# Perception4D/LidarSlam

Measured on AMD Instinct MI355X. Metric: LiDAR frames/sec (AddFrame end-to-end), VLS-128 scan, higher is better.
Workload: dtype f32+f64; 1 GPU; VLS-128 synthetic spinning scan, street canyon, 5 m/s, EgoMotion=MOTION_EXTRAPOLATION_AND_REGISTRATION, Undistortion=REFINED, library defaults; points_per_frame=255802, sequences=1, parallelism=1 sequence per GPU x 1, frames_resident_in_hbm=False

## Files before the change

### lidarslam_amd/csrc/lsa_accum.h

```cpp
#pragma once
#include "lsa_ctx.h"

namespace lsa
{

struct RotConst
{
  double R[9], dRx[9], dRy[9], dRz[9];
  double t[3];
};
struct RecordSet
{
  const double* rec[3];
  const uint8_t* status[3];
  int count[3];
  int cap[3];
  double sat2[3];
};
struct AccumConst
{
  RotConst rot;
  RecordSet set;
  int jac;
};
// ... 60 lines not shown
  const double s = (r0 * r0 + r1 * r1) + r2 * r2;
  double rho0, rho1;
  if (s <= a2)
  {
    const double value = 1.0 - s / a2;
    const double value_sq = value * value;
    rho0 = a2 / 3.0 * (1.0 - value_sq * value);
    rho1 = value_sq;
  }
  else { rho0 = a2 / 3.0; rho1 = 0.0; }
  rho0 *= weight; rho1 *= weight;
  acc[0] += 0.5 * rho0;
  acc[28] += 1.0;
  if (!jac) return;
  double J[3][6];
#pragma unroll
  for (int a = 0; a < 3; ++a)
#pragma unroll
    for (int b = 0; b < 3; ++b) J[a][b] = A[a * 3 + b];
  double vx, vy, vz, cx, cy, cz;
  mv3(c.dRx, Xx, Xy, Xz, vx, vy, vz); mv3(A, vx, vy, vz, cx, cy, cz); J[0][3] = cx; J[1][3] = cy; J[2][3] = cz;
  mv3(c.dRy, Xx, Xy, Xz, vx, vy, vz); mv3(A, vx, vy, vz, cx, cy, cz); J[0][4] = cx; J[1][4] = cy; J[2][4] = cz;
  mv3(c.dRz, Xx, Xy, Xz, vx, vy, vz); mv3(A, vx, vy, vz, cx, cy, cz); J[0][5] = cx; J[1][5] = cy; J[2][5] = cz;
  int h = 7;
#pragma unroll
  for (int a = 0; a < 6; ++a)
  {
    acc[1 + a] += rho1 * ((J[0][a] * r0 + J[1][a] * r1) + J[2][a] * r2);
#pragma unroll
    for (int b = a; b < 6; ++b) acc[h++] += rho1 * ((J[0][a] * J[0][b] + J[1][a] * J[1][b]) + J[2][a] * J[2][b]);
  }
}

__device__ __forceinline__ void accumulate_records(const RecordSet& rs, const RotConst& c, bool jac, int first, int stride, double acc[kAccumVals])
{
  const int total = rs.count[0] + rs.count[1] + rs.count[2];
  for (int gidx = first; gidx < total; gidx += stride)
  {
    int t = 0, i = gidx;
    if (i >= rs.count[0]) { i -= rs.count[0]; t = 1; if (i >= rs.count[1]) { i -= rs.count[1]; t = 2; } }
    if (rs.status[t][i] != LSA_MATCH_SUCCESS) continue;
    const double* rec = rs.rec[t];
    const size_t cap = (size_t)rs.cap[t];
    double A[9];
#pragma unroll
    for (int f = 0; f < 9; ++f) A[f] = rec[f * cap + i];
    const double Px = rec[9 * cap + i], Py = rec[10 * cap + i], Pz = rec[11 * cap + i];
    const double Xx = rec[12 * cap + i], Xy = rec[13 * cap + i], Xz = rec[14 * cap + i];
    const double weight = rec[15 * cap + i];
    accumulate_one(A, Px, Py, Pz, Xx, Xy, Xz, weight, rs.sat2[t], c, jac, acc);
  }
}

struct RecordRegs
{
  double v[16];
  double a2;
  int state;
};
__device__ __forceinline__ void record_load(const RecordSet& rs, int gidx, RecordRegs& r)
{
  const int total = rs.count[0] + rs.count[1] + rs.count[2];
  r.state = -1;
  r.a2 = 0.;
#pragma unroll
  for (int f = 0; f < 16; ++f) r.v[f] = 0.;
  if (gidx >= total) return;
  int t = 0, i = gidx;
  if (i >= rs.count[0]) { i -= rs.count[0]; t = 1; if (i >= rs.count[1]) { i -= rs.count[1]; t = 2; } }
  const double* rec = rs.rec[t];
  const size_t cap = (size_t)rs.cap[t];
  const uint8_t st = rs.status[t][i];
#pragma unroll
  for (int f = 0; f < 16; ++f) r.v[f] = rec[f * cap + i];
  r.a2 = rs.sat2[t];
  r.state = st == LSA_MATCH_SUCCESS ? 1 : 0;
}
__device__ __forceinline__ void record_stash(const RecordRegs& r, double* __restrict__ cache, int cstride, int at)
{
  if (r.state == 1)
  {
#pragma unroll
    for (int f = 0; f < 16; ++f) cache[f * cstride + at] = r.v[f];
    cache[16 * cstride + at] = r.a2;
  }
  else if (r.state == 0)
    cache[15 * cstride + at] = -1.;
}

__device__ __forceinline__ void accumulate_records_cached(const RecordSet& rs, const RotConst& c, int first, int stride, double* __restrict__ cache,
                                                          int cslots, int cstride, bool fill, int prefilled, double acc[kAccumVals])
{
  const int total = rs.count[0] + rs.count[1] + rs.count[2];
  int j = 0;
  for (int gidx = first; gidx < total; gidx += stride, ++j)
  {
    double A[9], Px, Py, Pz, Xx, Xy, Xz, weight, a2;
    const int at = j * (int)blockDim.x + (int)threadIdx.x;
    if (j < cslots && (!fill || j < prefilled))
    {
      weight = cache[15 * cstride + at];
      if (weight < 0.) continue;
#pragma unroll
      for (int f = 0; f < 9; ++f) A[f] = cache[f * cstride + at];
      Px = cache[9 * cstride + at]; Py = cache[10 * cstride + at]; Pz = cache[11 * cstride + at];
      Xx = cache[12 * cstride + at]; Xy = cache[13 * cstride + at]; Xz = cache[14 * cstride + at];
      a2 = cache[16 * cstride + at];
    }
    else
    {
      int t = 0, i = gidx;
      if (i >= rs.count[0]) { i -= rs.count[0]; t = 1; if (i >= rs.count[1]) { i -= rs.count[1]; t = 2; } }
      if (rs.status[t][i] != LSA_MATCH_SUCCESS)
      {
        if (j < cslots) cache[15 * cstride + at] = -1.;
        continue;
      }
      const double* rec = rs.rec[t];
      const size_t cap = (size_t)rs.cap[t];
#pragma unroll
      for (int f = 0; f < 9; ++f) A[f] = rec[f * cap + i];
      Px = rec[9 * cap + i]; Py = rec[10 * cap + i]; Pz = rec[11 * cap + i];
      Xx = rec[12 * cap + i]; Xy = rec[13 * cap + i]; Xz = rec[14 * cap + i];
      weight = rec[15 * cap + i];
      a2 = rs.sat2[t];
      if (j < cslots)
      {
#pragma unroll
        for (int f = 0; f < 9; ++f) cache[f * cstride + at] = A[f];
// ... 64 lines not shown
```

### lidarslam_amd/csrc/lsa_lm.hip

```cpp
#include <chrono>
#include <cmath>
#include "lsa_accum.h"
#include "lsa_device_math.h"
#include "lsa_sensor_terms.h"
#include "../../include/lsa_pmath.h"

using namespace lsa;

namespace
{

typedef unsigned long long u64;
#ifndef LSA_RECORD_PREFETCH
#define LSA_RECORD_PREFETCH 1
#endif
constexpr bool kRecordPrefetch = LSA_RECORD_PREFETCH != 0;

struct LmParams
{
  RecordSet set;
  double x0[6];
  int two_d;
  int max_iter;
  int min_matches;
  unsigned tag_base;
  int cslots;
  int give_up_block;
  const IcpLinkBlock* link;
  IcpLinkBlock* leave;
  int link_refine;
  int motion_from_args;
  posemath::ScanPoseClock clock;
  Rigid previous_world;
  double motion0[16];
  double* motion_dev;
  lsa_sensor_terms_t sensors;
  int sensors_on;
};

constexpr int kResPose = 0, kResInitial = 6, kResFinal = 7, kResSums = 8, kResSuccessful = 37, kResUnsuccessful = 38, kResIterations = 39,
              kResEvaluations = 40, kResSkipped = 41, kResCode = 42, kResMatches = 43, kResFailed = 44, kResCount = 45;
static_assert(kResCount <= kLmOut, "result does not fit the mailbox");

__device__ __forceinline__ constexpr int hidx(int a, int b) { return 7 + a * 6 - (a * (a - 1)) / 2 + (b - a); }
__device__ __forceinline__ constexpr int hsym(int a, int b) { return a <= b ? hidx(a, b) : hidx(b, a); }

struct LmState
{
  int cur_buf;
  double x[6], scale[6], diag[6];
  double radius, decrease_factor, x_norm, model_cost_change, delta_norm, initial_cost;
  int reuse_diagonal, consecutive_invalid, iter;
  int evaluations, successful, unsuccessful, iterations, code, skipped, matches;
};

struct Shared
{
  double wsum[kLmThreads / 64][kAccumVals];
  double part[kAccumVals][8];
  double sums[2][kAccumVals];
  double Hs[36], gs[6];
  double w[6];
  double rot[39];
  LmState lm;
  int failed;
  int stop;
  unsigned long long lap[6], tk;
  unsigned long long sub[4], st0;
};

__device__ __forceinline__ double uniform(double v)
{
  const long long b = __double_as_longlong(v);
  const int lo = __builtin_amdgcn_readfirstlane((int)(b & 0xffffffffll)), hi = __builtin_amdgcn_readfirstlane((int)(b >> 32));
  return __longlong_as_double(((long long)hi << 32) | (long long)(unsigned)lo);
}

__device__ __forceinline__ double lane_value(double v, int lane)
{
  const long long b = __double_as_longlong(v);
  const int lo = __shfl((int)(b & 0xffffffffll), lane), hi = __shfl((int)(b >> 32), lane);
  return __longlong_as_double(((long long)hi << 32) | (long long)(unsigned)lo);
}

__device__ __forceinline__ double lane_bcast(double v, int src)
{
  const long long b = __double_as_longlong(v);
  const int lo = __builtin_amdgcn_readlane((int)(b & 0xffffffffll), src), hi = __builtin_amdgcn_readlane((int)(b >> 32), src);
  return __longlong_as_double(((long long)hi << 32) | (long long)(unsigned)lo);
}

__device__ __forceinline__ void lm_lap(Shared& sh, int slot)
{
  if (threadIdx.x == 0)
  {
    const unsigned long long now = wall_clock64();
    sh.lap[slot] += now - sh.tk;
    sh.tk = now;
  }
}

__device__ __noinline__ void lm_sensor_terms(const lsa_sensor_terms_t* terms, Shared& sh)
{
  sensor_terms_add(*terms, sh.w, sh.rot, sh.rot + 9, sh.rot + 18, sh.rot + 27, true, sh.sums[1 - sh.lm.cur_buf]);
}

__device__ __forceinline__ bool lm_evaluate(const LmParams& p, unsigned epoch, u64* __restrict__ xchg, Shared& sh, double* __restrict__ cache, bool trace)
{
  {
    RotConst c;
#pragma unroll
    for (int i = 0; i < 9; ++i) { c.R[i] = uniform(sh.rot[i]); c.dRx[i] = uniform(sh.rot[9 + i]); c.dRy[i] = uniform(sh.rot[18 + i]); c.dRz[i] = uniform(sh.rot[27 + i]); }
#pragma unroll
    for (int i = 0; i < 3; ++i) c.t[i] = uniform(sh.rot[36 + i]);
    double acc[kAccumVals];
#pragma unroll
    for (int v = 0; v < kAccumVals; ++v) acc[v] = 0.;
    const unsigned long long e0 = trace ? wall_clock64() : 0ull;
    accumulate_records_cached(p.set, c, blockIdx.x * blockDim.x + threadIdx.x, gridDim.x * blockDim.x, cache, p.cslots, p.cslots * kLmThreads, epoch == 1, kRecordPrefetch && p.cslots > 0 ? 1 : 0, acc);
    const unsigned long long e1 = trace ? wall_clock64() : 0ull;
    int slot;
    const double total = wave_reduce_accum(acc, slot);
    if (trace && threadIdx.x == 0) { sh.lap[4] += e1 - e0; }
    if ((threadIdx.x & 1) == 0 && slot < kAccumVals) sh.wsum[threadIdx.x >> 6][slot] = total;
  }
  if (threadIdx.x == 0) sh.failed = 0;
  __syncthreads();
  if (trace) lm_lap(sh, 0);
  const unsigned tag = p.tag_base + epoch;
  const int nb = gridDim.x;
  u64* slots = xchg + (size_t)(epoch & 1u) * kLmBlocksMax * kMailboxStride;
  if (threadIdx.x < 2 * kAccumVals)
  {
    const int v = threadIdx.x >> 1, half = threadIdx.x & 1;
    double r = sh.wsum[0][v];
#pragma unroll
    for (int w = 1; w < kLmThreads / 64; ++w) r += sh.wsum[w][v];
    const u64 bits = (u64)__double_as_longlong(r);
    const unsigned word = half ? (unsigned)(bits >> 32) : (unsigned)(bits & 0xffffffffull);
    __hip_atomic_store(slots + (size_t)blockIdx.x * kMailboxStride + threadIdx.x, ((u64)tag << 32) | word, __ATOMIC_RELAXED, __HIP_MEMORY_SCOPE_AGENT);
  }
  static_assert(kLmThreads / 64 == 8, "a wavefront per partial sum of the fold");
// ... 318 lines not shown
    {
      cand[lm_act<N>(a)] = x[lm_act<N>(a)] + step[a] * scale[a];
      const double e = x[lm_act<N>(a)] - cand[lm_act<N>(a)];
      dn += e * e;
    }
    delta_norm = __builtin_sqrt(dn);
    ++evaluations;
    break;
  }

  if (lane < N) lm.diag[lane] = diag_row;
  if (l0)
  {
    if (use_tot && !first)
    {
#pragma unroll
      for (int a = 0; a < 6; ++a) lm.x[a] = x[a];
    }
    lm.cur_buf = cur_buf;
    lm.x_norm = x_norm; lm.radius = radius; lm.decrease_factor = decrease_factor;
    lm.model_cost_change = model_cost_change; lm.delta_norm = delta_norm;
    lm.reuse_diagonal = reuse_diagonal; lm.consecutive_invalid = consecutive_invalid;
    lm.iter = iter; lm.iterations = iter;
    lm.successful = successful; lm.unsuccessful = unsuccessful; lm.evaluations = evaluations;
    lm.code = code;
    sh.stop = code != kCodeNone ? 1 : 0;
  }
  stamp(3);
  return code != kCodeNone;
}

__device__ void leave_link(const LmParams& p, const LmState& lm, bool failed, int part)
{
  using namespace posemath;
  IcpLinkBlock* g = p.leave;
  const int lane = threadIdx.x & 63;
  const bool go = !failed && !lm.skipped && lm.successful != 1;
  if (!go)
  {
    if (lane == 0 && part == 0) g->go = 0ull;
    return;
  }
  if (part == 1 && !p.link_refine) return;
  const double half = lm.x[3 + (lane < 6 ? lane % 3 : 0)] * 0.5;
  const double v = lane < 3 ? lsa_cos(half) : lsa_sin(half);
  const double cx = lane_value(v, 0), cy = lane_value(v, 1), cz = lane_value(v, 2);
  const double sx = lane_value(v, 3), sy = lane_value(v, 4), sz = lane_value(v, 5);
  double x[6];
#pragma unroll
  for (int a = 0; a < 6; ++a) x[a] = lm.x[a];
  const Pose T = FromXYZRPYTrig(x, cx, sx, cy, sy, cz, sz);
  if (part == 0)
  {
    if (lane != 0) return;
    double x0[6];
    ToXYZRPY(T, x0);
    g->in.pose = ToRigid(T);
#pragma unroll
    for (int a = 0; a < 6; ++a) g->in.x0[a] = x0[a];
    g->go = 1ull;
    return;
  }
  WithinFrameMotion m;
  double mv[16];
#pragma unroll
  for (int i = 0; i < 16; ++i) mv[i] = p.motion0[i];
  if (!p.motion_from_args)
  {
#pragma unroll
    for (int i = 0; i < 16; ++i) mv[i] = p.motion_dev[i];
  }
  m.Time0 = mv[0]; m.Time1 = mv[1];
  m.Rot0 = {mv[2], mv[3], mv[4], mv[5]};
  m.Rot1 = {mv[6], mv[7], mv[8], mv[9]};
#pragma unroll
  for (int i = 0; i < 3; ++i) { m.Trans0[i] = mv[10 + i]; m.Trans1[i] = mv[13 + i]; }
  const Pose previous = FromRigid(p.previous_world);
  const Pose mine = InterpolateScanPose(p.clock, previous, T, lane == 1 ? m.Time1 : m.Time0);
  Pose worldToBaseEnd = Pose::Identity();
#pragma unroll
  for (int i = 0; i < 3; ++i)
#pragma unroll
    for (int j = 0; j < 4; ++j) worldToBaseEnd(i, j) = lane_value(mine(i, j), 1);
  if (lane != 0) return;
  Pose d0, d1;
  RefineUndistortionFrom(m, mine, worldToBaseEnd, T, d0, d1);
  g->in.ic = MakeInterpConst(d0, d1, m.Time0, m.Time1);
  double* o = p.motion_dev;
  o[0] = m.Time0; o[1] = m.Time1;
  o[2] = m.Rot0.w; o[3] = m.Rot0.x; o[4] = m.Rot0.y; o[5] = m.Rot0.z;
  o[6] = m.Rot1.w; o[7] = m.Rot1.x; o[8] = m.Rot1.y; o[9] = m.Rot1.z;
#pragma unroll
  for (int i = 0; i < 3; ++i) { o[10 + i] = m.Trans0[i]; o[13 + i] = m.Trans1[i]; }
}

__global__ __launch_bounds__(kLmThreads) void k_lm_solve(LmParams p, u64* __restrict__ xchg, u64* __restrict__ mailbox, unsigned out_tag, unsigned long long* trace)
{
  __shared__ Shared sh;
  extern __shared__ double lm_cache[];
  const bool tr = trace != nullptr && blockIdx.x == 0;
  RecordRegs pre;
  if (kRecordPrefetch && p.cslots > 0) record_load(p.set, blockIdx.x * blockDim.x + threadIdx.x, pre);
  if (p.link)
  {
    if (p.link->go != 1ull)
    {
      if (p.leave && blockIdx.x == 0 && threadIdx.x == 0) p.leave->go = 0ull;
      return;
    }
  }
  if (threadIdx.x < 64)
  {
    double x0[6];
#pragma unroll
    for (int a = 0; a < 6; ++a) x0[a] = p.x0[a];
    if (p.link)
    {
#pragma unroll
      for (int a = 0; a < 6; ++a) x0[a] = p.link->in.x0[a];
    }
    if (threadIdx.x == 0)
    {
      for (int i = 0; i < 6; ++i) sh.lap[i] = 0;
      for (int i = 0; i < 4; ++i) sh.sub[i] = 0;
      sh.st0 = 0;
      sh.tk = wall_clock64();
      sh.lap[5] = sh.tk;
      LmState& lm = sh.lm;
#pragma unroll
      for (int v = 0; v < kAccumVals; ++v) sh.sums[0][v] = 0.;
      lm.cur_buf = 0;
#pragma unroll
      for (int a = 0; a < 6; ++a) { lm.x[a] = x0[a]; lm.scale[a] = 1.; lm.diag[a] = 0.; }
      lm.radius = 1e4; lm.decrease_factor = 2.0; lm.x_norm = 0.; lm.model_cost_change = 0.; lm.delta_norm = 0.; lm.initial_cost = 0.;
      lm.reuse_diagonal = 0; lm.consecutive_invalid = 0; lm.iter = 0;
      lm.evaluations = 1; lm.successful = 0; lm.unsuccessful = 0; lm.iterations = 0; lm.code = kCodeNone; lm.skipped = 0; lm.matches = 0;
      sh.stop = 0;
    }
    finish_point(sh, x0[0], x0[1], x0[2], x0[3], x0[4], x0[5]);
  }
  if (kRecordPrefetch && p.cslots > 0) record_stash(pre, lm_cache, p.cslots * kLmThreads, threadIdx.x);
  __syncthreads();
  bool failed = false;
  for (unsigned epoch = 1;; ++epoch)
  {
    if (!lm_evaluate(p, epoch, xchg, sh, lm_cache, tr)) { failed = true; break; }
    if (threadIdx.x < 64)
    {
      if (threadIdx.x == 0 && tr) sh.st0 = wall_clock64();
      double cand[6];
      const bool stop = p.two_d ? lm_step<3>(p, sh, epoch == 1, cand) : lm_step<6>(p, sh, epoch == 1, cand);
      if (!stop) finish_point(sh, cand[0], cand[1], cand[2], cand[3], cand[4], cand[5]);
    }
    __syncthreads();
    if (tr) lm_lap(sh, 3);
    if (sh.stop) break;
  }
  if (blockIdx.x != 0) return;
  if (tr && threadIdx.x == 0)
  {
    for (int i = 0; i < 4; ++i) trace[i] += sh.lap[i];
    trace[4] += (unsigned long long)sh.lm.evaluations;
    trace[5] += wall_clock64() - sh.lap[5];
    trace[6] += 1;
    trace[7] += sh.lap[4];
    for (int i = 0; i < 4; ++i) trace[8 + i] += sh.sub[i];
  }
  if (p.leave && threadIdx.x >= 64 && threadIdx.x < 192) leave_link(p, sh.lm, failed, (threadIdx.x >> 6) - 1);
  if (threadIdx.x < 2 * kResCount)
  {
    const LmState& lm = sh.lm;
    const int v = threadIdx.x >> 1, half = threadIdx.x & 1;
// ... 525 lines not shown
```

### lidarslam_amd/csrc/lsa_match_fused.hip

```cpp
#include <cmath>
#include "lsa_knn.h"
#include "lsa_match_internal.h"

using namespace lsa;

namespace
{

constexpr int kPending = -2;
constexpr int kShells = 7;
#ifndef LSA_KFILL
#define LSA_KFILL 3
#endif
#ifndef LSA_KHEAVY
#define LSA_KHEAVY 192
#endif
constexpr int kFill = LSA_KFILL;
constexpr int kHeavyCandidates = LSA_KHEAVY;

__device__ __forceinline__ constexpr int shell_level(int s) { return s < 2 ? 0 : (s < 4 ? 1 : 2); }
__device__ __forceinline__ constexpr int shell_r(int s) { return s == 6 ? 3 : ((s & 1) ? 2 : 1); }

template <int G>
__device__ __forceinline__ unsigned group_sum(unsigned v)
// ... 250 lines not shown
        const float dx = qx - cur[u].x, dy = qy - cur[u].y, dz = qz - cur[u].z;
        L.insert(make_key((dx * dx + dy * dy) + dz * dz, __float_as_int(cur[u].w)));
      }
  }
  if (route)
  {
    atomicAdd(&route[2], walked);
    atomicMax(&route[5], walked);
  }
}

template <int KMAX>
__device__ __forceinline__ void scan_heavy_blocks(unsigned long long pending, int G, const RowTable tb, knn_key* save, const float4* s0, const float4* s1,
                                               const float4* s2, int cur, int cbase, int nent, unsigned cand, float qx, float qy, float qz, int k, int* route)
{
  const int tid = threadIdx.x, lane = tid & 63;
  while (pending)
  {
    const int lead = __ffsll((long long)pending) - 1;
    pending &= pending - 1;
    const int hcur = __shfl(cur, lead), hbase = __shfl(cbase, lead), hnent = __shfl(nent, lead);
    const unsigned hcand = (unsigned)__shfl((int)cand, lead);
    const float hx = __shfl(qx, lead), hy = __shfl(qy, lead), hz = __shfl(qz, lead);
    const float4* hsorted = hcur < 2 ? s0 : (hcur < 4 ? s1 : s2);
    knn_key* const hslot = save + (size_t)(((tid & ~63) + lead) / G) * KMAX;
    LaneList<KMAX> H;
    H.reset();
    scan_rows<KMAX, 64>(H, tb, hbase, hnent, hcand, lane, hsorted, hx, hy, hz, nullptr);
#pragma unroll
    for (int s = 0; s < KMAX; ++s)
    {
      knn_key m = kKeyEmpty;
      if (s < k)
      {
        m = H.v[0];
        group_min<64>(m);
        if (H.v[0] == m)
        {
#pragma unroll
          for (int j = 0; j + 1 < KMAX; ++j) H.v[j] = H.v[j + 1];
          H.v[KMAX - 1] = kKeyEmpty;
        }
      }
      if (lane == 0) hslot[s] = m;
    }
    if (route && lane == 0) atomicAdd(&route[2], (int)hcand);
  }
  asm volatile("s_waitcnt lgkmcnt(0)" ::: "memory");
}

enum { kOutNone = 0, kOutFound = 1, kOutFar = 2, kOutTail = 3 };

template <int KMAX, int G>
__device__ __forceinline__ int group_search(const GridDesc* __restrict__ desc, const GridPtrs& gp, float qx, float qy, float qz, int k, float far_d2,
                                            bool active, int gl, int tid, const RowTable& tb, knn_key* save, knn_key (&best)[KMAX], float& ub_out, int* route,
                                            unsigned long long* phase = nullptr)
{
  auto stamp = [&](int i) { if (phase && (tid & 63) == 0) phase[(tid >> 6) * 8 + i] = wall_clock64(); };
  constexpr int E1 = (9 + G - 1) / G, E2 = (25 + G - 1) / G, E3 = (49 + G - 1) / G;
  constexpr int CAP = table_capacity<G>();
  static_assert((256 / G) * CAP <= kTableEntries, "row tables");
  const int gbase = ((tid - gl) / G) * CAP;
  const int base3[3] = {gbase, gbase + G * E1 + 1, gbase + G * (E1 + E2) + 2};
  const GridDesc g0 = desc[0], g1 = desc[1], g2 = desc[2];
  LevelView v0, v1, v2;
  level_view(v0, g0, qx, qy, qz);
  level_view(v1, g1, qx, qy, qz);
  level_view(v2, g2, qx, qy, qz);
  auto bound2 = [&](int s) {
    const int l = shell_level(s), r = shell_r(s);
    return l == 0 ? proven2(g0, v0, r) : (l == 1 ? proven2(g1, v1, r) : proven2(g2, v2, r));
  };
  auto fetch_any = [&](int s, bool live, bool& covered) -> unsigned {
    const int l = shell_level(s), r = shell_r(s);
    const GridDesc& g = l == 0 ? g0 : (l == 1 ? g1 : g2);
    const LevelView& v = l == 0 ? v0 : (l == 1 ? v1 : v2);
    const uint32_t* cs = l == 0 ? gp.cell_start[0] : (l == 1 ? gp.cell_start[1] : gp.cell_start[2]);
    uint32_t b[E3], en[E3];
    shell_rows<G, E3>(g, cs, v, r, gl, live, b, en, covered);
    return store_rows<G, E3>(tb, gbase, gl, live, b, en);
  };

  int outcome = kOutNone;
  int sh = -1, base = gbase;
  unsigned total = 0;
  bool sh_covered = false;
  bool need = active;
  ub_out = INFINITY;

  unsigned tot3[3];
  {
    uint32_t b0[E1], e0[E1], b1[E2], e1[E2], b2[E1], e2[E1];
    bool c0, c1, c2;
    shell_rows<G, E1>(g0, gp.cell_start[0], v0, 1, gl, active, b0, e0, c0);
    shell_rows<G, E2>(g0, gp.cell_start[0], v0, 2, gl, active, b1, e1, c1);
    shell_rows<G, E1>(g1, gp.cell_start[1], v1, 1, gl, active, b2, e2, c2);
    tot3[0] = store_rows<G, E1>(tb, base3[0], gl, active, b0, e0);
    tot3[1] = store_rows<G, E2>(tb, base3[1], gl, active, b1, e1);
    tot3[2] = store_rows<G, E1>(tb, base3[2], gl, active, b2, e2);
    const bool cov[3] = {c0, c1, c2};
#pragma unroll
    for (int j = 0; j < 3; ++j)
      if (need && !cov[j] && (tot3[j] & 0xfffffu) < (unsigned)k && bound2(j) > far_d2)
      {
        outcome = kOutFar;
        need = false;
      }
    auto choose = [&](int j) {
      sh = j; sh_covered = cov[j]; base = base3[j]; total = tot3[j];
      need = false;
    };
#pragma unroll
    for (int j = 0; j < 3; ++j)
      if (need && (cov[j] || (tot3[j] & 0xfffffu) >= (unsigned)(kFill * k))) choose(j);
#pragma unroll
    for (int j = 2; j >= 0; --j)
      if (need && (tot3[j] & 0xfffffu) >= (unsigned)k) choose(j);
// ... 353 lines not shown
          for (int b = 0; b < 3; ++b) A[a * 3 + b] = ((V[a][0] * d0) * V[b][0] + (V[a][1] * d1) * V[b][1]) + (V[a][2] * d2) * V[b][2];
        if (!isfinite(A[0]) || !isfinite(d0 * d1 * d2)) st = LSA_MATCH_INVALID_NUMERICAL;
        else w = 1.0;
      }
    }
    if (st == LSA_MATCH_SUCCESS) write_record(rec, cap, i, A, mean, (double)q4.x, (double)q4.y, (double)q4.z, w);
  }
  if (st != LSA_MATCH_SUCCESS) rec[(size_t)15 * cap + i] = 0.;
  return st;
}

template <int KMAX>
__device__ __forceinline__ void search_whole_target(const float4* __restrict__ sorted, int npoints, float qx, float qy, float qz, int k, knn_key (&best)[KMAX])
{
  const int lane = threadIdx.x & 63;
  LaneList<KMAX> L;
  L.reset();
  for (int c = lane; c < npoints; c += 64)
  {
    const float4 p = sorted[c];
    const float dx = qx - p.x, dy = qy - p.y, dz = qz - p.z;
    L.insert(make_key((dx * dx + dy * dy) + dz * dz, __float_as_int(p.w)));
  }
  merge_lists<KMAX, 64>(L, k, best);
}

__device__ __forceinline__ bool load_inputs(const FusedArgs& a, IcpInputs& gin)
{
  __shared__ unsigned long long go;
  if (a.link)
  {
    constexpr int words = (int)(sizeof(IcpInputs) / 8);
    static_assert(words + 1 <= 256 && offsetof(IcpLinkBlock, in) == 8, "one word per thread, go in front");
    const unsigned long long* src = reinterpret_cast<const unsigned long long*>(a.link);
    if ((int)threadIdx.x < words) reinterpret_cast<unsigned long long*>(&gin)[threadIdx.x] = src[1 + threadIdx.x];
    else if ((int)threadIdx.x == words) go = src[0];
  }
  else if (threadIdx.x == 0)
  {
    go = 1ull;
    gin.pose = a.pose;
    if (a.undistort) gin.ic = a.ic;
  }
  __syncthreads();
  return go == 1ull;
}

template <int KMAX, int G, int TYPE, bool FUSE, int KC>
__device__ __forceinline__ void search_type(const FusedArgs& a, IcpInputs& gin, const FusedType& t, int block, SearchShared& sh, FitStage<256 / G, KC>& fs)
{
  constexpr int QB = 256 / G;
  const int tid = threadIdx.x, gl = tid % G, ql = tid / G;
  const int q = block * QB + ql;
  const bool active = q < t.nq;
  float4 q4 = {0.f, 0.f, 0.f, 0.f}, b4 = {0.f, 0.f, 0.f, 0.f};
  if (active)
  {
    q4 = t.queries[2 * (size_t)q];
    if (a.undistort) b4 = t.queries[2 * (size_t)q + 1];
  }
  if (!load_inputs(a, gin)) return;
  const Rigid& pose = gin.pose;
  const InterpConst* const ic = a.undistort ? &gin.ic : nullptr;
  if (t.route_stats)
  {
    if (tid < 6) sh.route[tid] = 0;
    if (tid < 32) sh.phase[tid] = 0;
    __syncthreads();
  }
  float qx = 0.f, qy = 0.f, qz = 0.f;
  if (active)
  {
    auto place = [&](const Rigid& P, const InterpConst* C) {
      if (C)
      {
        Rigid U;
        interp_eval(*C, __hiloint2double(__float_as_int(b4.y), __float_as_int(b4.x)), U);
        double ux, uy, uz;
        rigid_apply(U, (double)q4.x, (double)q4.y, (double)q4.z, ux, uy, uz);
        q4.x = (float)ux; q4.y = (float)uy; q4.z = (float)uz;
        if (gl == 0) const_cast<float4*>(t.queries)[2 * (size_t)q] = q4;
      }
      double wx, wy, wz;
      rigid_apply(P, (double)q4.x, (double)q4.y, (double)q4.z, wx, wy, wz);
      qx = (float)wx; qy = (float)wy; qz = (float)wz;
    };
    place(pose, ic);
    if constexpr (FUSE) { if (gl == 0) fs.q4[ql] = q4; }
  }
  knn_key best[KMAX];
#pragma unroll
  for (int s = 0; s < KMAX; ++s) best[s] = kKeyEmpty;
  float ub = INFINITY;
  const unsigned long long tick0 = t.trace ? wall_clock64() : 0ull;
  const RowTable tb = {sh.b, sh.e, sh.p};
  const int outcome = group_search<KMAX, G>(t.desc, t.gp, qx, qy, qz, t.k, t.far_d2, active, gl, tid, tb, sh.save, best, ub, t.route_stats ? sh.route : nullptr, t.trace ? sh.phase : nullptr);
  int cnt = 0;
#pragma unroll
  for (int s = 0; s < KMAX; ++s)
    if (s < t.k && best[s] != kKeyEmpty) ++cnt;
  const unsigned long long tick1 = t.trace ? wall_clock64() : 0ull;
  if constexpr (FUSE)
  {
    const bool tail = active && outcome == kOutTail;
    if (tail && gl == 0) fs.pre[ql] = kStagePending;
    group_stage<KMAX, TYPE, G, QB, KC>(best, outcome == kOutFar ? kKnnFar : cnt, t.mc, t.xyzl, gl, ql, active && !tail, true, fs);
    if (t.trace && (tid & 63) == 0) sh.phase[(tid >> 6) * 8 + 4] = wall_clock64();
    __syncthreads();
    if (tid >= 64) return;
    if (t.trace && tid == 0) sh.phase[5] = wall_clock64();
    const int lane = tid;
    if (lane < LSA_MATCH_NSTATUS) fs.lh[lane] = 0;
    const int i = block * QB + lane;
    const bool have = lane < QB && i < t.nq;
    unsigned long long pending = __ballot(have && fs.pre[lane < QB ? lane : 0] == kStagePending);
    while (pending)
    {
      const int src = __ffsll((long long)pending) - 1;
      pending &= pending - 1;
      const float4 b4 = fs.q4[src];
      double wx, wy, wz;
      rigid_apply(pose, (double)b4.x, (double)b4.y, (double)b4.z, wx, wy, wz);
      search_whole_target<KMAX>(t.gp.sorted[0], t.npoints, (float)wx, (float)wy, (float)wz, t.k, best);
      int c2 = 0;
#pragma unroll
      for (int s = 0; s < KMAX; ++s)
        if (s < t.k && best[s] != kKeyEmpty) ++c2;
      group_stage<KMAX, TYPE, G, QB, KC>(best, c2, t.mc, t.xyzl, gl, src, true, lane < G, fs);
      if (lane == 0) atomicAdd(t.hist + LSA_MATCH_NSTATUS, 1);
      asm volatile("s_waitcnt lgkmcnt(0)" ::: "memory");
    }
    if (have)
    {
#ifdef LSA_ABLATE_FINISH
      const int st = fs.pre[lane] == LSA_MATCH_SUCCESS ? LSA_MATCH_MSE_TOO_LARGE : fs.pre[lane];
#else
      const int st = finish_model<TYPE, QB, KC>(fs, lane, t.mc, t.rec, t.cap, i);
#endif
      t.status[i] = (uint8_t)st;
      atomicAdd(&fs.lh[st], 1);
    }
    asm volatile("s_waitcnt lgkmcnt(0)" ::: "memory");
    if (lane < LSA_MATCH_NSTATUS && fs.lh[lane]) atomicAdd(&t.hist[lane], fs.lh[lane]);
  }
  if (!FUSE && gl == 0 && active)
  {
#pragma unroll
    for (int s = 0; s < KMAX; ++s)
      if (s < t.k)
// ... 48 lines not shown
  __syncthreads();
  const int i = block * QPB + tid;
  const bool have = tid < QPB && i < t.nq;
  int n = 0;
  if (have && !t.mc.bad_param) n = t.knn_cnt[i];
  unsigned long long pending = __ballot(have && n == kPending);
  while (pending)
  {
    const int src = __ffsll((long long)pending) - 1;
    pending &= pending - 1;
    const int qi = block * QPB + (tid - lane) + src;
    const float4 q4 = t.queries[2 * (size_t)qi];
    double wx, wy, wz;
    rigid_apply(pose, (double)q4.x, (double)q4.y, (double)q4.z, wx, wy, wz);
    knn_key best[KMAX];
    search_whole_target<KMAX>(t.gp.sorted[0], t.npoints, (float)wx, (float)wy, (float)wz, t.k, best);
    if (lane == src)
    {
      int cnt = 0;
#pragma unroll
      for (int s = 0; s < KMAX; ++s)
        if (s < t.k)
        {
          t.knn_idx[(size_t)s * t.cap + qi] = key_idx(best[s]);
          t.knn_d2[(size_t)s * t.cap + qi] = key_d2(best[s]);
          if (best[s] != kKeyEmpty) ++cnt;
        }
      n = cnt;
      atomicAdd(t.hist + LSA_MATCH_NSTATUS, 1);
    }
  }
  if (have)
  {
    const int st = fit_model<KMAX, TYPE>(
      t.queries[2 * (size_t)i], t.mc, n, [&](int s) { return t.knn_idx[(size_t)s * t.cap + i]; }, [&](int s) { return t.knn_d2[(size_t)s * t.cap + i]; },
      t.xyzl, sh.nb, sh.nd, QPB, tid, t.rec, t.cap, i);
    t.status[i] = (uint8_t)st;
    atomicAdd(&sh.lh[st], 1);
  }
  __syncthreads();
  if (tid < LSA_MATCH_NSTATUS && sh.lh[tid]) atomicAdd(&t.hist[tid], sh.lh[tid]);
}

template <int KE, int KP, int KB, bool FUSE>
__global__ __launch_bounds__(256, 4) void k_search_all(FusedArgs a)
{
  constexpr int QB = 256 / kGE;
  constexpr int KC = FUSE ? (KE > KP ? (KE > KB ? KE : KB) : (KP > KB ? KP : KB)) : 1;
  static_assert(kGE == kGP && kGP == kGB, "one workgroup serves 256 / G keypoints of any type");
  __shared__ SearchShared sh;
  __shared__ FitStage<QB, KC> fs;
  __shared__ IcpInputs gin;
  const int xcd = blockIdx.x % 8, j = blockIdx.x / 8;
  const int se = (a.t[0].nblocks + 7) / 8, sp = (a.t[1].nblocks + 7) / 8;
  if (j < se)
  {
    const int block = xcd * se + j;
    if (block >= a.t[0].nblocks) return;
    search_type<KE, kGE, LSA_EDGE, FUSE, KC>(a, gin, a.t[0], block, sh, fs);
  }
  else if (j < se + sp)
  {
    const int block = xcd * sp + (j - se);
    if (block >= a.t[1].nblocks) return;
    search_type<KP, kGP, LSA_PLANE, FUSE, KC>(a, gin, a.t[1], block, sh, fs);
  }
  else
  {
    if constexpr (KB > 0)
    {
      const int sb = (a.t[2].nblocks + 7) / 8;
      const int block = xcd * sb + (j - se - sp);
      if (block >= a.t[2].nblocks) return;
      search_type<KB, kGB, LSA_BLOB, FUSE, KC>(a, gin, a.t[2], block, sh, fs);
    }
  }
}

template <int KE, int KP, int KB>
__global__ __launch_bounds__(kModelBlock) void k_model_all(FusedArgs a)
{
  __shared__ ModelShared<KE, kModelBlock> sh;
  if (a.link && a.link->go != 1ull) return;
  int b = blockIdx.x;
  if (b < a.t[0].mblocks) { model_type<KE, LSA_EDGE, kModelBlock>(a.pose, a.t[0], b, sh); return; }
  b -= a.t[0].mblocks;
  if (b < a.t[1].mblocks) { model_type<KP, LSA_PLANE, kModelBlock>(a.pose, a.t[1], b, sh); return; }
  b -= a.t[1].mblocks;
  if constexpr (KB > 0) model_type<KB, LSA_BLOB, kModelBlock>(a.pose, a.t[2], b, sh);
}

template <int KE, int KP, int KB>
void launch_fused(lsa_ctx* ctx, const FusedArgs& a, double search_bytes, double model_bytes, hipStream_t st)
{
  const int grid = 8 * ((a.t[0].nblocks + 7) / 8 + (a.t[1].nblocks + 7) / 8 + (a.t[2].nblocks + 7) / 8);
  if (a.fuse_model)
  {
    ProfScope ps(ctx, "match_search_model", search_bytes + model_bytes, st);
    hipLaunchKernelGGL((k_search_all<KE, KP, KB, true>), dim3(grid), dim3(256), 0, st, a);
    return;
  }
  if (grid > 0)
  {
    ProfScope ps(ctx, "match_search", search_bytes, st);
    hipLaunchKernelGGL((k_search_all<KE, KP, KB, false>), dim3(grid), dim3(256), 0, st, a);
  }
  ProfScope ps(ctx, "match_model", model_bytes, st);
  hipLaunchKernelGGL((k_model_all<KE, KP, KB>), dim3(a.t[0].mblocks + a.t[1].mblocks + a.t[2].mblocks), dim3(kModelBlock), 0, st, a);
}

}

namespace lsa
{

int enqueue_fused_match(lsa_ctx* ctx, const MatchPrep* preps, int count, const double pose[16], hipStream_t st, const InterpConst* undistort, int link, bool link_undistorts)
{
  FusedArgs a;
  std::memset(&a, 0, sizeof(a));
  if (link >= 0) a.link = reinterpret_cast<const IcpLinkBlock*>(ctx->link_dev + (size_t)link * kLinkWords);
  else row_major_to_rt(pose, a.pose.R, a.pose.t);
  int kmax[3] = {1, 1, 1};
  const int lanes[3] = {kGE, kGP, kGB};
  double search_bytes = 0, model_bytes = 0;
  for (int i = 0; i < count; ++i)
  {
// ... 52 lines not shown
```

### lidarslam_amd/csrc/lsa_posemath.h

```cpp
#pragma once
#include "../../include/lsa_pmath.h"

#if defined(__HIPCC__)
#define LSA_HDM __host__ __device__
#else
#define LSA_HDM
#endif

namespace lsa
{

struct Rigid
{
  double R[9];
  double t[3];
};

struct InterpConst
{
  double qa[4], qb[4];
  double d, theta, sin_theta;
  double trans0[3], trans1[3];
  double time0, time1;
  Rigid h0;
// ... 168 lines not shown
{
  w[0] = p(0, 3); w[1] = p(1, 3); w[2] = p(2, 3);
  w[3] = lsa_atan2(p(2, 1), p(2, 2));
  w[4] = -lsa_asin(p(2, 0));
  w[5] = lsa_atan2(p(1, 0), p(0, 0));
}

LSA_HD Pose LinearInterpolation(const Pose& H0, const Pose& H1, double t, double t0, double t1)
{
  if (t0 == t1 || IsApprox(H0, H1)) return H1;
  const double time = (t - t0) / (t1 - t0);
  Pose r = Pose::Identity();
  SetRotation(r, Slerp(ToQuaternion(H0), ToQuaternion(H1), time));
  for (int i = 0; i < 3; ++i) r(i, 3) = H0(i, 3) + time * (H1(i, 3) - H0(i, 3));
  return r;
}

LSA_HD double RotationAngle(const Pose& p)
{
  const Quaternion q = ToQuaternion(p);
  const double n = __builtin_sqrt((q.x * q.x + q.y * q.y) + q.z * q.z);
  return (n != 0.) ? 2. * lsa_atan2(n, __builtin_fabs(q.w)) : 0.;
}

struct WithinFrameMotion
{
  double Time0 = 0., Time1 = 1.;
  Quaternion Rot0{1, 0, 0, 0}, Rot1{1, 0, 0, 0};
  double Trans0[3] = {0, 0, 0}, Trans1[3] = {0, 0, 0};
  LSA_HDM Pose GetH0() const
  {
    Pose p = Pose::Identity();
    SetRotation(p, Rot0);
    for (int i = 0; i < 3; ++i) p(i, 3) = Trans0[i];
    return p;
  }
  LSA_HDM Pose GetH1() const
  {
    Pose p = Pose::Identity();
    SetRotation(p, Rot1);
    for (int i = 0; i < 3; ++i) p(i, 3) = Trans1[i];
    return p;
  }
  LSA_HDM void SetTransforms(const Pose& H0, const Pose& H1)
  {
    Rot0 = ToQuaternion(H0);
    Rot1 = ToQuaternion(H1);
    for (int i = 0; i < 3; ++i) { Trans0[i] = H0(i, 3); Trans1[i] = H1(i, 3); }
  }
  LSA_HDM void SetTimes(double t0, double t1) { Time0 = t0; Time1 = t1; }
  LSA_HDM double GetTimeRange() const { return Time1 - Time0; }
};

LSA_HD InterpConst MakeInterpConst(const Pose& H0, const Pose& H1, double t0, double t1)
{
  InterpConst c;
  for (int i = 0; i < 3; ++i) { c.trans0[i] = H0(i, 3); c.trans1[i] = H1(i, 3); }
  const Quaternion qa = ToQuaternion(H0), qb = ToQuaternion(H1);
  c.qa[0] = qa.w; c.qa[1] = qa.x; c.qa[2] = qa.y; c.qa[3] = qa.z;
  c.qb[0] = qb.w; c.qb[1] = qb.x; c.qb[2] = qb.y; c.qb[3] = qb.z;
  c.time0 = t0; c.time1 = t1;
  Pose G0 = Pose::Identity(), G1 = Pose::Identity();
  SetRotation(G0, qa);
  SetRotation(G1, qb);
  for (int i = 0; i < 3; ++i)
  {
    for (int j = 0; j < 3; ++j) c.h0.R[i * 3 + j] = G0(i, j);
    c.h0.t[i] = c.trans0[i];
  }
  double d = 0, na = 1, nb = 1;
  for (int i = 0; i < 3; ++i)
    for (int j = 0; j < 3; ++j) { const double e = G0(i, j) - G1(i, j); d += e * e; na += G0(i, j) * G0(i, j); nb += G1(i, j) * G1(i, j); }
  for (int i = 0; i < 3; ++i) { const double e = c.trans0[i] - c.trans1[i]; d += e * e; na += c.trans0[i] * c.trans0[i]; nb += c.trans1[i] * c.trans1[i]; }
  const bool approx = d <= 1e-12 * 1e-12 * (nb < na ? nb : na);
  c.invalid = (t0 == t1 || approx) ? 1 : 0;
  c.d = (c.qa[1] * c.qb[1] + c.qa[3] * c.qb[3]) + (c.qa[2] * c.qb[2] + c.qa[0] * c.qb[0]);
  const double absD = __builtin_fabs(c.d);
  c.linear = absD >= kOneMinusEps ? 1 : 0;
  c.theta = c.linear ? 0.0 : lsa_acos(absD);
  c.sin_theta = c.linear ? 1.0 : lsa_sin(c.theta);
  return c;
}

struct ScanPoseClock
{
  int have_log;
  double prev_time;
  double cur_time;
  double max_ratio;
};
LSA_HD Pose InterpolateScanPose(const ScanPoseClock& k, const Pose& previousTworld, const Pose& tworld, double time)
{
  if (!k.have_log) return tworld;
  if (__builtin_fabs(time / (k.cur_time - k.prev_time)) > k.max_ratio) return tworld;
  return LinearInterpolation(previousTworld, tworld, k.cur_time + time, k.prev_time, k.cur_time);
}
LSA_HD void RefineUndistortionFrom(WithinFrameMotion& motion, const Pose& worldToBaseBegin, const Pose& worldToBaseEnd, const Pose& tworld, Pose& d0, Pose& d1)
{
  const Pose previousBaseBegin = motion.GetH0();
  const Pose previousBaseEnd = motion.GetH1();
  const Pose baseToWorld = Inverse(tworld);
  const Pose newBaseBegin = baseToWorld * worldToBaseBegin;
  const Pose newBaseEnd = baseToWorld * worldToBaseEnd;
  motion.SetTransforms(newBaseBegin, newBaseEnd);
  d0 = newBaseBegin * Inverse(previousBaseBegin);
  d1 = newBaseEnd * Inverse(previousBaseEnd);
}
LSA_HD void RefineUndistortion(WithinFrameMotion& motion, const ScanPoseClock& k, const Pose& previousTworld, const Pose& tworld, Pose& d0, Pose& d1)
{
  const Pose worldToBaseBegin = InterpolateScanPose(k, previousTworld, tworld, motion.Time0);
  const Pose worldToBaseEnd = InterpolateScanPose(k, previousTworld, tworld, motion.Time1);
  RefineUndistortionFrom(motion, worldToBaseBegin, worldToBaseEnd, tworld, d0, d1);
}

}
}
```

Before: 1372 frames/s.

## Spread per-link pose math across lanes and hoist scalar loads in LM and match kernels

```diff
diff --git a/lidarslam_amd/csrc/lsa_accum.h b/lidarslam_amd/csrc/lsa_accum.h
--- a/lidarslam_amd/csrc/lsa_accum.h
+++ b/lidarslam_amd/csrc/lsa_accum.h
@@ -136,29 +136,49 @@
   }
 }
 
+struct RecordType
+{
+  const double* rec;
+  const uint8_t* status;
+  size_t cap;
+  double sat2;
+};
+__device__ __forceinline__ RecordType record_type(const RecordSet& rs, int t)
+{
+  const double *r0 = rs.rec[0], *r1 = rs.rec[1], *r2 = rs.rec[2];
+  const uint8_t *s0 = rs.status[0], *s1 = rs.status[1], *s2 = rs.status[2];
+  const int c0 = rs.cap[0], c1 = rs.cap[1], c2 = rs.cap[2];
+  const double a0 = rs.sat2[0], a1 = rs.sat2[1], a2 = rs.sat2[2];
+  RecordType y;
+  y.rec = t == 0 ? r0 : (t == 1 ? r1 : r2);
+  y.status = t == 0 ? s0 : (t == 1 ? s1 : s2);
+  y.cap = (size_t)(t == 0 ? c0 : (t == 1 ? c1 : c2));
+  y.sat2 = t == 0 ? a0 : (t == 1 ? a1 : a2);
+  return y;
+}
+
 struct RecordRegs
 {
   double v[16];
   double a2;
   int state;
 };
-__device__ __forceinline__ void record_load(const RecordSet& rs, int gidx, RecordRegs& r)
+__device__ __forceinline__ void record_load(const RecordSet& rs, int gidx, const void* spare, RecordRegs& r)
 {
   const int total = rs.count[0] + rs.count[1] + rs.count[2];
-  r.state = -1;
-  r.a2 = 0.;
-#pragma unroll
-  for (int f = 0; f < 16; ++f) r.v[f] = 0.;
-  if (gidx >= total) return;
-  int t = 0, i = gidx;
+  const bool any = total > 0, mine = gidx < total;
+  int t = 0, i = mine ? gidx : total - 1;
   if (i >= rs.count[0]) { i -= rs.count[0]; t = 1; if (i >= rs.count[1]) { i -= rs.count[1]; t = 2; } }
-  const double* rec = rs.rec[t];
-  const size_t cap = (size_t)rs.cap[t];
-  const uint8_t st = rs.status[t][i];
+  const RecordType y = record_type(rs, t);
+  const double* rec = any ? y.rec : static_cast<const double*>(spare);
+  const uint8_t* status = any ? y.status : static_cast<const uint8_t*>(spare);
+  const size_t cap = any ? y.cap : (size_t)0;
+  i = any ? i : 0;
+  const uint8_t st = status[i];
 #pragma unroll
   for (int f = 0; f < 16; ++f) r.v[f] = rec[f * cap + i];
-  r.a2 = rs.sat2[t];
-  r.state = st == LSA_MATCH_SUCCESS ? 1 : 0;
+  r.a2 = y.sat2;
+  r.state = !mine ? -1 : (st == LSA_MATCH_SUCCESS ? 1 : 0);
 }
 __device__ __forceinline__ void record_stash(const RecordRegs& r, double* __restrict__ cache, int cstride, int at)
 {
diff --git a/lidarslam_amd/csrc/lsa_lm.hip b/lidarslam_amd/csrc/lsa_lm.hip
--- a/lidarslam_amd/csrc/lsa_lm.hip
+++ b/lidarslam_amd/csrc/lsa_lm.hip
@@ -38,6 +38,8 @@
   int sensors_on;
 };
 
+constexpr int kLinkX0Word = (int)((offsetof(IcpLinkBlock, in) + offsetof(IcpInputs, x0)) / 8);
+
 constexpr int kResPose = 0, kResInitial = 6, kResFinal = 7, kResSums = 8, kResSuccessful = 37, kResUnsuccessful = 38, kResIterations = 39,
               kResEvaluations = 40, kResSkipped = 41, kResCode = 42, kResMatches = 43, kResFailed = 44, kResCount = 45;
 static_assert(kResCount <= kLmOut, "result does not fit the mailbox");
@@ -88,6 +90,12 @@
   const long long b = __double_as_longlong(v);
   const int lo = __builtin_amdgcn_readlane((int)(b & 0xffffffffll), src), hi = __builtin_amdgcn_readlane((int)(b >> 32), src);
   return __longlong_as_double(((long long)hi << 32) | (long long)(unsigned)lo);
+}
+
+__device__ __forceinline__ u64 lane_bcast_u64(u64 v, int src)
+{
+  const unsigned lo = (unsigned)__builtin_amdgcn_readlane((int)(v & 0xffffffffull), src), hi = (unsigned)__builtin_amdgcn_readlane((int)(v >> 32), src);
+  return ((u64)hi << 32) | lo;
 }
 
 __device__ __forceinline__ void lm_lap(Shared& sh, int slot)
@@ -512,9 +520,10 @@
   const Pose T = FromXYZRPYTrig(x, cx, sx, cy, sy, cz, sz);
   if (part == 0)
   {
+    const double angle = lsa_atan2(lane == 1 ? T(1, 0) : T(2, 1), lane == 1 ? T(0, 0) : T(2, 2));
+    const double yaw = lane_value(angle, 1);
     if (lane != 0) return;
-    double x0[6];
-    ToXYZRPY(T, x0);
+    const double x0[6] = {T(0, 3), T(1, 3), T(2, 3), angle, -lsa_asin(T(2, 0)), yaw};
     g->in.pose = ToRigid(T);
 #pragma unroll
     for (int a = 0; a < 6; ++a) g->in.x0[a] = x0[a];
@@ -535,23 +544,35 @@
   m.Rot1 = {mv[6], mv[7], mv[8], mv[9]};
 #pragma unroll
   for (int i = 0; i < 3; ++i) { m.Trans0[i] = mv[10 + i]; m.Trans1[i] = mv[13 + i]; }
+  const bool end = lane == 1;
   const Pose previous = FromRigid(p.previous_world);
-  const Pose mine = InterpolateScanPose(p.clock, previous, T, lane == 1 ? m.Time1 : m.Time0);
-  Pose worldToBaseEnd = Pose::Identity();
+  const Pose mine = InterpolateScanPose(p.clock, previous, T, end ? m.Time1 : m.Time0);
+  const Quaternion rot = {end ? m.Rot1.w : m.Rot0.w, end ? m.Rot1.x : m.Rot0.x, end ? m.Rot1.y : m.Rot0.y, end ? m.Rot1.z : m.Rot0.z};
+  const double trans[3] = {end ? m.Trans1[0] : m.Trans0[0], end ? m.Trans1[1] : m.Trans0[1], end ? m.Trans1[2] : m.Trans0[2]};
+  Pose newBase, d;
+  RefineUndistortionEnd(rot, trans, mine, T, newBase, d);
+  const Quaternion newRot = ToQuaternion(newBase);
+  const InterpEnd e0 = MakeInterpEnd(d);
+  InterpEnd e1;
+  e1.G = Pose::Identity();
 #pragma unroll
   for (int i = 0; i < 3; ++i)
-#pragma unroll
-    for (int j = 0; j < 4; ++j) worldToBaseEnd(i, j) = lane_value(mine(i, j), 1);
+  {
+    e1.trans[i] = lane_value(e0.trans[i], 1);
+#pragma unroll
+    for (int j = 0; j < 3; ++j) e1.G(i, j) = lane_value(e0.G(i, j), 1);
+  }
+  e1.q = {lane_value(e0.q.w, 1), lane_value(e0.q.x, 1), lane_value(e0.q.y, 1), lane_value(e0.q.z, 1)};
+  const Quaternion newRot1 = {lane_value(newRot.w, 1), lane_value(newRot.x, 1), lane_value(newRot.y, 1), lane_value(newRot.z, 1)};
+  const double newTrans1[3] = {lane_value(newBase(0, 3), 1), lane_value(newBase(1, 3), 1), lane_value(newBase(2, 3), 1)};
   if (lane != 0) return;
-  Pose d0, d1;
-  RefineUndistortionFrom(m, mine, worldToBaseEnd, T, d0, d1);
-  g->in.ic = MakeInterpConst(d0, d1, m.Time0, m.Time1);
+  g->in.ic = JoinInterpEnds(e0, e1, m.Time0, m.Time1);
   double* o = p.motion_dev;
   o[0] = m.Time0; o[1] = m.Time1;
-  o[2] = m.Rot0.w; o[3] = m.Rot0.x; o[4] = m.Rot0.y; o[5] = m.Rot0.z;
-  o[6] = m.Rot1.w; o[7] = m.Rot1.x; o[8] = m.Rot1.y; o[9] = m.Rot1.z;
-#pragma unroll
-  for (int i = 0; i < 3; ++i) { o[10 + i] = m.Trans0[i]; o[13 + i] = m.Trans1[i]; }
+  o[2] = newRot.w; o[3] = newRot.x; o[4] = newRot.y; o[5] = newRot.z;
+  o[6] = newRot1.w; o[7] = newRot1.x; o[8] = newRot1.y; o[9] = newRot1.z;
+#pragma unroll
+  for (int i = 0; i < 3; ++i) { o[10 + i] = newBase(i, 3); o[13 + i] = newTrans1[i]; }
 }
 
 __global__ __launch_bounds__(kLmThreads) void k_lm_solve(LmParams p, u64* __restrict__ xchg, u64* __restrict__ mailbox, unsigned out_tag, unsigned long long* trace)
@@ -559,13 +580,18 @@
   __shared__ Shared sh;
   extern __shared__ double lm_cache[];
   const bool tr = trace != nullptr && blockIdx.x == 0;
+  const int lane = threadIdx.x & 63;
+  const IcpLinkBlock* const link = p.link;
+  IcpLinkBlock* const leave = p.leave;
+  u64 link_word = 0ull;
+  if (link) link_word = reinterpret_cast<const u64*>(link)[lane < 6 ? kLinkX0Word + lane : 0];
   RecordRegs pre;
-  if (kRecordPrefetch && p.cslots > 0) record_load(p.set, blockIdx.x * blockDim.x + threadIdx.x, pre);
-  if (p.link)
-  {
-    if (p.link->go != 1ull)
-    {
-      if (p.leave && blockIdx.x == 0 && threadIdx.x == 0) p.leave->go = 0ull;
+  if (kRecordPrefetch) record_load(p.set, blockIdx.x * blockDim.x + threadIdx.x, xchg, pre);
+  if (link)
+  {
+    if (lane_bcast_u64(link_word, 6) != 1ull)
+    {
+      if (leave && blockIdx.x == 0 && threadIdx.x == 0) leave->go = 0ull;
       return;
     }
   }
@@ -574,10 +600,10 @@
     double x0[6];
 #pragma unroll
     for (int a = 0; a < 6; ++a) x0[a] = p.x0[a];
-    if (p.link)
-    {
-#pragma unroll
-      for (int a = 0; a < 6; ++a) x0[a] = p.link->in.x0[a];
+    if (link)
+    {
+#pragma unroll
+      for (int a = 0; a < 6; ++a) x0[a] = __longlong_as_double((long long)lane_bcast_u64(link_word, a));
     }
     if (threadIdx.x == 0)
     {
diff --git a/lidarslam_amd/csrc/lsa_match_fused.hip b/lidarslam_amd/csrc/lsa_match_fused.hip
--- a/lidarslam_amd/csrc/lsa_match_fused.hip
+++ b/lidarslam_amd/csrc/lsa_match_fused.hip
@@ -326,7 +326,7 @@
 enum { kOutNone = 0, kOutFound = 1, kOutFar = 2, kOutTail = 3 };
 
 template <int KMAX, int G>
-__device__ __forceinline__ int group_search(const GridDesc* __restrict__ desc, const GridPtrs& gp, float qx, float qy, float qz, int k, float far_d2,
+__device__ __forceinline__ int group_search(const GridDesc& g0, const GridDesc& g1, const GridDesc& g2, const GridPtrs& gp, float qx, float qy, float qz, int k, float far_d2,
                                             bool active, int gl, int tid, const RowTable& tb, knn_key* save, knn_key (&best)[KMAX], float& ub_out, int* route,
                                             unsigned long long* phase = nullptr)
 {
@@ -336,7 +336,6 @@
   static_assert((256 / G) * CAP <= kTableEntries, "row tables");
   const int gbase = ((tid - gl) / G) * CAP;
   const int base3[3] = {gbase, gbase + G * E1 + 1, gbase + G * (E1 + E2) + 2};
-  const GridDesc g0 = desc[0], g1 = desc[1], g2 = desc[2];
   LevelView v0, v1, v2;
   level_view(v0, g0, qx, qy, qz);
   level_view(v1, g1, qx, qy, qz);
@@ -796,14 +795,19 @@
   constexpr int QB = 256 / G;
   const int tid = threadIdx.x, gl = tid % G, ql = tid / G;
   const int q = block * QB + ql;
-  const bool active = q < t.nq;
-  float4 q4 = {0.f, 0.f, 0.f, 0.f}, b4 = {0.f, 0.f, 0.f, 0.f};
-  if (active)
-  {
-    q4 = t.queries[2 * (size_t)q];
-    if (a.undistort) b4 = t.queries[2 * (size_t)q + 1];
-  }
+  const int nq = t.nq;
+  const float4* const queries = t.queries;
+  const GridDesc* const desc = t.desc;
+  asm volatile("" ::"s"(nq), "s"(queries), "s"(desc), "s"(a.undistort), "s"(a.link));
+  const bool active = q < nq;
+  float4 q4, b4 = {0.f, 0.f, 0.f, 0.f};
+  const size_t qs = (size_t)(active ? q : nq - 1);
+  q4 = queries[2 * qs];
+  if (a.undistort) b4 = queries[2 * qs + 1];
+  const GridDesc g0 = desc[0], g1 = desc[1], g2 = desc[2];
   if (!load_inputs(a, gin)) return;
+  asm volatile("" : "+v"(q4.x), "+v"(q4.y), "+v"(q4.z), "+v"(q4.w), "+v"(b4.x), "+v"(b4.y));
+  if (!active) q4 = {0.f, 0.f, 0.f, 0.f};
   const Rigid& pose = gin.pose;
   const InterpConst* const ic = a.undistort ? &gin.ic : nullptr;
   if (t.route_stats)
@@ -838,7 +842,7 @@
   float ub = INFINITY;
   const unsigned long long tick0 = t.trace ? wall_clock64() : 0ull;
   const RowTable tb = {sh.b, sh.e, sh.p};
-  const int outcome = group_search<KMAX, G>(t.desc, t.gp, qx, qy, qz, t.k, t.far_d2, active, gl, tid, tb, sh.save, best, ub, t.route_stats ? sh.route : nullptr, t.trace ? sh.phase : nullptr);
+  const int outcome = group_search<KMAX, G>(g0, g1, g2, t.gp, qx, qy, qz, t.k, t.far_d2, active, gl, tid, tb, sh.save, best, ub, t.route_stats ? sh.route : nullptr, t.trace ? sh.phase : nullptr);
   int cnt = 0;
 #pragma unroll
   for (int s = 0; s < KMAX; ++s)
@@ -993,26 +997,28 @@
   __shared__ FitStage<QB, KC> fs;
   __shared__ IcpInputs gin;
   const int xcd = blockIdx.x % 8, j = blockIdx.x / 8;
-  const int se = (a.t[0].nblocks + 7) / 8, sp = (a.t[1].nblocks + 7) / 8;
+  const int nbe = a.t[0].nblocks, nbp = a.t[1].nblocks, nbb = KB > 0 ? a.t[2].nblocks : 0;
+  asm volatile("" ::"s"(nbe), "s"(nbp), "s"(nbb));
+  const int se = (nbe + 7) / 8, sp = (nbp + 7) / 8;
   if (j < se)
   {
     const int block = xcd * se + j;
-    if (block >= a.t[0].nblocks) return;
+    if (block >= nbe) return;
     search_type<KE, kGE, LSA_EDGE, FUSE, KC>(a, gin, a.t[0], block, sh, fs);
   }
   else if (j < se + sp)
   {
     const int block = xcd * sp + (j - se);
-    if (block >= a.t[1].nblocks) return;
+    if (block >= nbp) return;
     search_type<KP, kGP, LSA_PLANE, FUSE, KC>(a, gin, a.t[1], block, sh, fs);
   }
   else
   {
     if constexpr (KB > 0)
     {
-      const int sb = (a.t[2].nblocks + 7) / 8;
+      const int sb = (nbb + 7) / 8;
       const int block = xcd * sb + (j - se - sp);
-      if (block >= a.t[2].nblocks) return;
+      if (block >= nbb) return;
       search_type<KB, kGB, LSA_BLOB, FUSE, KC>(a, gin, a.t[2], block, sh, fs);
     }
   }
diff --git a/lidarslam_amd/csrc/lsa_posemath.h b/lidarslam_amd/csrc/lsa_posemath.h
--- a/lidarslam_amd/csrc/lsa_posemath.h
+++ b/lidarslam_amd/csrc/lsa_posemath.h
@@ -244,17 +244,31 @@
   LSA_HDM double GetTimeRange() const { return Time1 - Time0; }
 };
 
-LSA_HD InterpConst MakeInterpConst(const Pose& H0, const Pose& H1, double t0, double t1)
+struct InterpEnd
+{
+  double trans[3];
+  Quaternion q;
+  Pose G;
+};
+LSA_HD InterpEnd MakeInterpEnd(const Pose& H)
+{
+  InterpEnd e;
+  for (int i = 0; i < 3; ++i) e.trans[i] = H(i, 3);
+  e.q = ToQuaternion(H);
+  e.G = Pose::Identity();
+  SetRotation(e.G, e.q);
+  return e;
+}
+LSA_HD InterpConst JoinInterpEnds(const InterpEnd& a, const InterpEnd& b, double t0, double t1)
 {
   InterpConst c;
-  for (int i = 0; i < 3; ++i) { c.trans0[i] = H0(i, 3); c.trans1[i] = H1(i, 3); }
-  const Quaternion qa = ToQuaternion(H0), qb = ToQuaternion(H1);
+  for (int i = 0; i < 3; ++i) { c.trans0[i] = a.trans[i]; c.trans1[i] = b.trans[i]; }
+  const Quaternion qa = a.q, qb = b.q;
   c.qa[0] = qa.w; c.qa[1] = qa.x; c.qa[2] = qa.y; c.qa[3] = qa.z;
   c.qb[0] = qb.w; c.qb[1] = qb.x; c.qb[2] = qb.y; c.qb[3] = qb.z;
   c.time0 = t0; c.time1 = t1;
-  Pose G0 = Pose::Identity(), G1 = Pose::Identity();
-  SetRotation(G0, qa);
-  SetRotation(G1, qb);
+  const Pose& G0 = a.G;
+  const Pose& G1 = b.G;
   for (int i = 0; i < 3; ++i)
   {
     for (int j = 0; j < 3; ++j) c.h0.R[i * 3 + j] = G0(i, j);
@@ -273,6 +287,10 @@
   c.sin_theta = c.linear ? 1.0 : lsa_sin(c.theta);
   return c;
 }
+LSA_HD InterpConst MakeInterpConst(const Pose& H0, const Pose& H1, double t0, double t1)
+{
+  return JoinInterpEnds(MakeInterpEnd(H0), MakeInterpEnd(H1), t0, t1);
+}
 
 struct ScanPoseClock
 {
@@ -287,16 +305,21 @@
   if (__builtin_fabs(time / (k.cur_time - k.prev_time)) > k.max_ratio) return tworld;
   return LinearInterpolation(previousTworld, tworld, k.cur_time + time, k.prev_time, k.cur_time);
 }
+LSA_HD void RefineUndistortionEnd(const Quaternion& previousRot, const double previousTrans[3], const Pose& worldToBase, const Pose& tworld, Pose& newBase, Pose& d)
+{
+  Pose previousBase = Pose::Identity();
+  SetRotation(previousBase, previousRot);
+  for (int i = 0; i < 3; ++i) previousBase(i, 3) = previousTrans[i];
+  const Pose baseToWorld = Inverse(tworld);
+  newBase = baseToWorld * worldToBase;
+  d = newBase * Inverse(previousBase);
+}
 LSA_HD void RefineUndistortionFrom(WithinFrameMotion& motion, const Pose& worldToBaseBegin, const Pose& worldToBaseEnd, const Pose& tworld, Pose& d0, Pose& d1)
 {
-  const Pose previousBaseBegin = motion.GetH0();
-  const Pose previousBaseEnd = motion.GetH1();
-  const Pose baseToWorld = Inverse(tworld);
-  const Pose newBaseBegin = baseToWorld * worldToBaseBegin;
-  const Pose newBaseEnd = baseToWorld * worldToBaseEnd;
+  Pose newBaseBegin, newBaseEnd;
+  RefineUndistortionEnd(motion.Rot0, motion.Trans0, worldToBaseBegin, tworld, newBaseBegin, d0);
+  RefineUndistortionEnd(motion.Rot1, motion.Trans1, worldToBaseEnd, tworld, newBaseEnd, d1);
   motion.SetTransforms(newBaseBegin, newBaseEnd);
-  d0 = newBaseBegin * Inverse(previousBaseBegin);
-  d1 = newBaseEnd * Inverse(previousBaseEnd);
 }
 LSA_HD void RefineUndistortion(WithinFrameMotion& motion, const ScanPoseClock& k, const Pose& previousTworld, const Pose& tworld, Pose& d0, Pose& d1)
 {
```

Result: no change. 1380 frames/s, median of 2 (+0.6%).
